# zoharl3/mantaflow

Measured on AMD Instinct MI355X. Metric: Mcells/s per step (advect+CG+FLIP), 256^3 grid, higher is better.
Workload: dtype f32; 1 GPU; 256^3 smoke step on 1 x MI355X: advectSemiLagrange(density, order 2) + advectSemiLagrange(vel, order 2) + setWallBcs + solvePressure (MIC-CG, cgAccuracy 1e-3); parallelism=single GPU

## Files before the change

### mantaflow_amd/csrc/pressure.hip

```cpp
#include "common.h"
#include "pressure.h"
#include <float.h>
#include <stdlib.h>
#include <stdio.h>
#include <type_traits>

using namespace mf;

static thread_local int g_last_shortcut[3] = {0, 0, 0};


__device__ __forceinline__ float wave_shr1(float v) {
	return __int_as_float(__builtin_amdgcn_update_dpp(__float_as_int(v), __float_as_int(v), 0x138, 0xf, 0xf, false));
}
__device__ __forceinline__ float wave_shl1(float v) {
	return __int_as_float(__builtin_amdgcn_update_dpp(__float_as_int(v), __float_as_int(v), 0x130, 0xf, 0xf, false));
}
__device__ __forceinline__ int4 unpack_flags(unsigned w) {
	return make_int4((w & 0x1u) ? MF_FLUID : 0, (w & 0x100u) ? MF_FLUID : 0, (w & 0x10000u) ? MF_FLUID : 0, (w & 0x1000000u) ? MF_FLUID : 0);
}
template <unsigned BIT>
__device__ __forceinline__ float4 unpack_coef(unsigned w) {
	return make_float4((w & BIT) ? -1.f : 0.f, (w & (BIT << 8)) ? -1.f : 0.f, (w & (BIT << 16)) ? -1.f : 0.f, (w & (BIT << 24)) ? -1.f : 0.f);
}
#ifndef AM_NT
#define AM_NT 2
#endif
#ifndef PCG_NT_MI
#define PCG_NT_MI 10
#endif
constexpr int64_t PCG_NT_CELLS = (int64_t)PCG_NT_MI << 20;
#ifndef AMP_NT
#define AMP_NT 1
#endif
template <bool DOT, bool IS3D, int R, bool PACKED>
__global__ void __launch_bounds__(BLOCK)
k_apply_matrix_v5(Dim d, const int32_t* __restrict__ flags, float* __restrict__ dst, const float* __restrict__ src,
                  const float* __restrict__ A0, const float* __restrict__ Ai, const float* __restrict__ Aj,
                  const float* __restrict__ Ak, double* __restrict__ partials, const CgScalars* __restrict__ sc, int jgroups, int tpb,
                  const unsigned char* __restrict__ pack, int dk0, int dk1, int a0p, const int* __restrict__ bempty = nullptr, int nbj = 0,
                  const int* __restrict__ outside_bad = nullptr, const int* __restrict__ xr = nullptr) {
	if (DOT && sc->done) return;
	const int qx = d.sx >> 2;
	const int64_t nthr = (int64_t)qx * jgroups * d.sz;
	const int vb0 = xcd_swizzle(blockIdx.x, gridDim.x) * tpb;
	double acc = 0.0;
#pragma unroll 1
	for (int t = 0; t < tpb; t++) {
	const int64_t T0 = (int64_t)(vb0 + t) * BLOCK + threadIdx.x;
	const bool live = T0 < nthr;
	const int64_t T = live ? T0 : nthr - 1;
	const int qi = (int)(T % qx);
	const int64_t rg = T / qx;
	const int j0 = (int)(rg % jgroups) * R;
	const int k = (int)(rg / jgroups);
	int q_lo = 0, q_hi = qx;
	if (IS3D && bempty && outside_bad[0] == 0) {
		if (xr) {
			q_lo = (xr[0] & ~7) >> 2;
			q_hi = ((xr[1] + 7) & ~7) >> 2;
		}
		if (bempty[(k >> 3) * nbj + (j0 >> 3)] || qi < q_lo || qi >= q_hi) continue;
	}
	const int lane = threadIdx.x & 63;
	const float4 z4 = make_float4(0.f, 0.f, 0.f, 0.f);
	const int64_t Y = d.Y, Z = d.Z;
	const int64_t row0 = ((int64_t)k * d.sy + j0) * d.sx + 4 * qi;
	int4 f[R];
	float4 sv[R + 2], ajv[R + 1], a0[R], ai[R], ak[R], akm[R], szm[R], szp[R];
	float sl[R], al[R], sr[R];
	{
		const int jm = (rg > 0) ? -1 : 0;
		sv[0] = *(const float4*)(src + row0 + jm * Y);
		if (PACKED) ajv[0] = unpack_coef<4u>(*(const unsigned*)(pack + row0 + jm * Y));
		else ajv[0] = *(const float4*)(Aj + row0 + jm * Y);
	}
#pragma unroll
	for (int r = 0; r < R; r++) {
		const int jr = (j0 + r < d.sy) ? r : (d.sy - 1 - j0);
		const int64_t idx = row0 + jr * Y;
		sv[r + 1] = ((AMP_NT & 1) && (!DOT || (a0p & 2))) ? ld_nt4(src + idx) : *(const float4*)(src + idx);
		unsigned pw = 0;
		if (PACKED) pw = *(const unsigned*)(pack + idx);
		if (PACKED && (a0p & 1)) a0[r] = make_float4((float)((pw >> 4) & 15u), (float)((pw >> 12) & 15u), (float)((pw >> 20) & 15u), (float)((pw >> 28) & 15u));
		else a0[r] = (AM_NT >= 1) ? ld_nt4(A0 + idx) : *(const float4*)(A0 + idx);
		if (PACKED) {
			f[r] = unpack_flags(pw);
			ajv[r + 1] = unpack_coef<4u>(pw);
			ai[r] = unpack_coef<2u>(pw);
		} else {
			f[r] = (AM_NT >= 1) ? ld_nt4i(flags + idx) : *(const int4*)(flags + idx);
			ajv[r + 1] = (AM_NT >= 3) ? ld_nt4(Aj + idx) : *(const float4*)(Aj + idx);
// ... 600 lines not shown
		else {
			lo = fminf(lo, fpart[2 * i]);
			hi = fmaxf(hi, fpart[2 * i + 1]);
		}
	}
	dd = strided_sum(dpart_dot, nbd);
	block_minmax(lo, hi);
	__syncthreads();
	ss = block_sum(ss);
	__syncthreads();
	dd = block_sum(dd);
	if (threadIdx.x == 0) {
		float resNorm;
		if (l2)
			resNorm = (float)ss;
		else {
			const float alo = fabsf(lo), ahi = fabsf(hi);
			resNorm = alo > ahi ? alo : ahi;
		}
		sc->resNorm = resNorm;
		if (resNorm < sc->accuracy) {
			sc->sigma = resNorm;
			sc->done = 1;
		} else {
			const float sigmaNew = (float)dd;
			sc->beta = sigmaNew / sc->sigma;
			sc->sigmaNew = sigmaNew;
			sc->sigma = sigmaNew;
			if (!((double)resNorm < 1e35)) {
				sc->diverged = 1;
			}
		}
	}
}
template <bool SKIP>
__global__ void __launch_bounds__(BLOCK)
k_cg_update_search_x(int64_t n, const CgScalars* __restrict__ sc, float* __restrict__ dst, float* __restrict__ search, const float* __restrict__ tmp,
                     const int* __restrict__ bempty = nullptr, int nbj = 0, int sx = 0, int sy = 0, const int* __restrict__ outside_bad = nullptr,
                     const int* __restrict__ xr = nullptr, int nt = 0) {
	if (!sc->xpending) return;
	const bool upd = !sc->done;
	const int xlo = (SKIP && xr) ? (xr[0] & ~7) : 0, xhi = (SKIP && xr) ? ((xr[1] + 7) & ~7) : 0x7fffffff;
	const float alpha = sc->alpha, beta = sc->beta;
	const int64_t n4 = n >> 2;
	const bool zero_outside = SKIP && outside_bad[0] == 0;
	for (int64_t q = blockIdx.x * (int64_t)BLOCK + threadIdx.x; q < n4; q += (int64_t)gridDim.x * BLOCK) {
		if (SKIP && zero_outside) {
			const int64_t row = (4 * q) / sx;
			const int j = (int)(row % sy), k = (int)(row / sy);
			const int xc = (int)(4 * q - row * sx);
			if (bempty[(k >> 3) * nbj + (j >> 3)] || xc < xlo || xc >= xhi) continue;
		}
		float4 s = nt ? ld_nt4(search + 4 * q) : ((float4*)search)[q];
		float4 x = nt ? ld_nt4(dst + 4 * q) : ((float4*)dst)[q];
		x.x = x.x + alpha * s.x; x.y = x.y + alpha * s.y; x.z = x.z + alpha * s.z; x.w = x.w + alpha * s.w;
		if (nt) st_nt4(dst + 4 * q, x);
		else ((float4*)dst)[q] = x;
		if (upd) {
			const float4 t = nt ? ld_nt4(tmp + 4 * q) : ((const float4*)tmp)[q];
			s.x = t.x + beta * s.x; s.y = t.y + beta * s.y; s.z = t.z + beta * s.z; s.w = t.w + beta * s.w;
			if (nt) st_nt4(search + 4 * q, s);
			else ((float4*)search)[q] = s;
		}
	}
	if (blockIdx.x == 0 && threadIdx.x < (n & 3)) {
		const int64_t i = (n4 << 2) + threadIdx.x;
		const float s = search[i];
		dst[i] = dst[i] + alpha * s;
		if (upd) search[i] = tmp[i] + beta * s;
	}
}

__global__ void __launch_bounds__(BLOCK)
k_cg_update_search_x_scalar(int64_t n, const CgScalars* __restrict__ sc, float* __restrict__ dst, float* __restrict__ search, const float* __restrict__ tmp) {
	if (!sc->xpending) return;
	const bool upd = !sc->done;
	const float alpha = sc->alpha, beta = sc->beta;
	for (int64_t i = blockIdx.x * (int64_t)BLOCK + threadIdx.x; i < n; i += (int64_t)gridDim.x * BLOCK) {
		const float s = search[i];
		dst[i] = dst[i] + alpha * s;
		if (upd) search[i] = tmp[i] + beta * s;
	}
}
__global__ void k_slab_alpha_x(const double* __restrict__ g, int world, CgScalars* __restrict__ sc, const int32_t* __restrict__ state) {
	if (state && state[0]) {
		sc->alpha = 0.f;
		sc->nalpha = -0.f;
		sc->xpending = 0;
		sc->done = 1;
		return;
	}
	double acc = 0.0;
	for (int r = 0; r < world; r++) acc += g[2 * r + 1];
	const float dp = (float)acc;
	const float a = (fabs((double)dp) > 0.) ? sc->sigma / dp : 0.f;
	sc->alpha = a;
	sc->nalpha = -a;
	sc->xpending = 1;
	sc->done = 0;
	sc->sigmaPrev = sc->sigma;
}
__global__ void __launch_bounds__(BLOCK)
k_slab_axpy_r(int64_t n, const double* __restrict__ g, int world, CgScalars* __restrict__ sc, const int32_t* __restrict__ state,
              float* __restrict__ residual, const float* __restrict__ tmp, float* __restrict__ fpart, int nt) {
	const bool stopped = state[0] != 0;
	float a = 0.f;
	if (!stopped) {
		double acc = 0.0;
		for (int r = 0; r < world; r++) acc += g[2 * r + 1];
		const float dp = (float)acc;
		a = (fabs((double)dp) > 0.) ? sc->sigma / dp : 0.f;
	}
	const float nalpha = -a;
	if (blockIdx.x == 0 && threadIdx.x == 0) {
		sc->alpha = a;
		sc->nalpha = nalpha;
		sc->xpending = stopped ? 0 : 1;
		sc->done = stopped ? 1 : 0;
		if (!stopped) sc->sigmaPrev = sc->sigma;
	}
	if (stopped) return;
	float lo = FLT_MAX, hi = -FLT_MAX;
	const int64_t n4 = n >> 2;
	for (int64_t q = blockIdx.x * (int64_t)BLOCK + threadIdx.x; q < n4; q += (int64_t)gridDim.x * BLOCK) {
		float4 r = ((float4*)residual)[q];
		const float4 t = nt ? ld_nt4(tmp + 4 * q) : ((const float4*)tmp)[q];
		r.x = r.x + nalpha * t.x; r.y = r.y + nalpha * t.y; r.z = r.z + nalpha * t.z; r.w = r.w + nalpha * t.w;
		((float4*)residual)[q] = r;
		lo = fminf(fminf(lo, r.x), fminf(r.y, fminf(r.z, r.w)));
		hi = fmaxf(fmaxf(hi, r.x), fmaxf(r.y, fmaxf(r.z, r.w)));
	}
	if (blockIdx.x == 0 && threadIdx.x < (n & 3)) {
		const int64_t i = (n4 << 2) + threadIdx.x;
		const float r = residual[i] + nalpha * tmp[i];
		residual[i] = r;
		lo = fminf(lo, r);
		hi = fmaxf(hi, r);
	}
	block_minmax(lo, hi);
	if (threadIdx.x == 0) {
		fpart[2 * blockIdx.x] = lo;
		fpart[2 * blockIdx.x + 1] = hi;
	}
}
__global__ void __launch_bounds__(BLOCK)
k_slab_axpy_r_scalar(int64_t n, const CgScalars* __restrict__ sc, float* __restrict__ residual, const float* __restrict__ tmp, float* __restrict__ fpart) {
	if (sc->done) return;
	const float nalpha = sc->nalpha;
	float lo = FLT_MAX, hi = -FLT_MAX;
	for (int64_t i = blockIdx.x * (int64_t)BLOCK + threadIdx.x; i < n; i += (int64_t)gridDim.x * BLOCK) {
		const float r = residual[i] + nalpha * tmp[i];
		residual[i] = r;
		lo = fminf(lo, r);
		hi = fmaxf(hi, r);
	}
	block_minmax(lo, hi);
	if (threadIdx.x == 0) {
		fpart[2 * blockIdx.x] = lo;
		fpart[2 * blockIdx.x + 1] = hi;
	}
}
__global__ void k_slab_beta_x(const double* __restrict__ g, int world, CgScalars* __restrict__ sc, float accuracy, int iter, int32_t* __restrict__ state) {
	if (state && state[0]) return;
	double acc = 0.0, mx = 0.0;
	for (int r = 0; r < world; r++) {
		acc += g[2 * r + 1];
		mx = g[2 * r] > mx ? g[2 * r] : mx;
	}
	const float sigmaNew = (float)acc;
	const float rn = (float)mx;
	sc->resNorm = rn;
	sc->beta = sigmaNew / sc->sigma;
	sc->sigma = sigmaNew;
	if (state) {
		if (rn < accuracy) {
			state[0] = 1;
			state[1] = iter;
			sc->done = 1;
		} else if (!(rn < 1e35f)) {
			state[0] = 2;
			state[1] = iter;
			sc->done = 1;
		}
	}
}
__global__ void __launch_bounds__(BLOCK)
k_slab_update_search_x(int64_t n, const double* __restrict__ g, int world, CgScalars* __restrict__ sc, float accuracy, int iter,
                       int32_t* __restrict__ state, float* __restrict__ dst, float* __restrict__ search, const float* __restrict__ tmp, int nt) {
	if (!sc->xpending) return;
	double acc = 0.0, mx = 0.0;
	for (int r = 0; r < world; r++) {
		acc += g[2 * r + 1];
		mx = g[2 * r] > mx ? g[2 * r] : mx;
	}
	const float sigmaNew = (float)acc;
	const float rn = (float)mx;
	const float beta = sigmaNew / sc->sigmaPrev;
	const bool converged = rn < accuracy, diverged = !converged && !(rn < 1e35f);
	if (blockIdx.x == 0 && threadIdx.x == 0) {
		sc->resNorm = rn;
		sc->beta = beta;
		sc->sigma = sigmaNew;
		if (converged || diverged) {
			state[0] = converged ? 1 : 2;
			state[1] = iter;
			sc->done = 1;
		}
	}
	const bool upd = !(converged || diverged);
	const float alpha = sc->alpha;
	const int64_t n4 = n >> 2;
	for (int64_t q = blockIdx.x * (int64_t)BLOCK + threadIdx.x; q < n4; q += (int64_t)gridDim.x * BLOCK) {
		float4 s = nt ? ld_nt4(search + 4 * q) : ((float4*)search)[q];
		float4 x = nt ? ld_nt4(dst + 4 * q) : ((float4*)dst)[q];
		x.x = x.x + alpha * s.x; x.y = x.y + alpha * s.y; x.z = x.z + alpha * s.z; x.w = x.w + alpha * s.w;
		if (nt) st_nt4(dst + 4 * q, x);
		else ((float4*)dst)[q] = x;
		if (upd) {
			const float4 t = nt ? ld_nt4(tmp + 4 * q) : ((const float4*)tmp)[q];
			s.x = t.x + beta * s.x; s.y = t.y + beta * s.y; s.z = t.z + beta * s.z; s.w = t.w + beta * s.w;
			if (nt) st_nt4(search + 4 * q, s);
			else ((float4*)search)[q] = s;
		}
	}
	if (blockIdx.x == 0 && threadIdx.x < (n & 3)) {
		const int64_t i = (n4 << 2) + threadIdx.x;
		const float s = search[i];
		dst[i] = dst[i] + alpha * s;
		if (upd) search[i] = tmp[i] + beta * s;
	}
}

__global__ void __launch_bounds__(BLOCK) k_fin_sum(int nb, const double* __restrict__ partials, double* __restrict__ out) {
	double acc = strided_sum(partials, nb);
	acc = block_sum(acc);
	if (threadIdx.x == 0) out[0] = acc;
}
__global__ void __launch_bounds__(BLOCK) k_fin_maxabs(int nb, const float* __restrict__ fpart, double* __restrict__ out) {
	float lo = FLT_MAX, hi = -FLT_MAX;
	for (int i = threadIdx.x; i < nb; i += blockDim.x) {
		lo = fminf(lo, fpart[2 * i]);
		hi = fmaxf(hi, fpart[2 * i + 1]);
	}
	block_minmax(lo, hi);
	if (threadIdx.x == 0) {
		const float alo = fabsf(lo), ahi = fabsf(hi);
		out[0] = (double)(alo > ahi ? alo : ahi);
	}
}

__global__ void __launch_bounds__(BLOCK)
k_diffusion_matrix(int64_t n, const int32_t* __restrict__ flags, float* __restrict__ A0, float* __restrict__ Ai, float* __restrict__ Aj,
                   float* __restrict__ Ak, float alpha) {
	const int64_t idx = blockIdx.x * (int64_t)BLOCK + threadIdx.x;
	if (idx >= n) return;
	if (flags[idx] & MF_OBSTACLE) {
		Ai[idx] = Aj[idx] = Ak[idx] = 0.f;
		A0[idx] = 1.f;
	} else {
		Ai[idx] *= alpha;
		Aj[idx] *= alpha;
		Ak[idx] *= alpha;
		A0[idx] = A0[idx] * alpha + 1.f;
	}
}

static int cg_solve_core(const Dim& d, const int32_t* flags, float* dst, const float* rhs, float* residual, float* search, float* tmp,
                         const float* A0, const float* Ai, const float* Aj, const float* Ak, float* Aprecond, int pc, float accuracy,
                         int maxIter, int useL2Norm, float* out_host, void* stream, const unsigned char* free_pack, const PcExternal* ext = nullptr);
__global__ void __launch_bounds__(BLOCK)
k_pad_system(int sx, int px, int64_t np_, const int32_t* __restrict__ flags, const float* __restrict__ rhs, const float* __restrict__ tmp,
             const float* __restrict__ A0, const float* __restrict__ Ai, const float* __restrict__ Aj, const float* __restrict__ Ak,
             int32_t* __restrict__ pf, float* __restrict__ pr, float* __restrict__ pt, float* __restrict__ p0, float* __restrict__ pi,
             float* __restrict__ pj, float* __restrict__ pk) {
	for (int64_t q = blockIdx.x * (int64_t)BLOCK + threadIdx.x; q < np_; q += (int64_t)gridDim.x * BLOCK) {
		const int64_t row = q / px;
		const int i = (int)(q - row * px);
		const bool in = i < sx;
		const int64_t s = row * sx + i;
		pf[q] = in ? flags[s] : MF_OBSTACLE;
		pr[q] = in ? rhs[s] : 0.f;
		pt[q] = in ? tmp[s] : 0.f;
		p0[q] = in ? A0[s] : 0.f;
		pi[q] = in ? Ai[s] : 0.f;
		pj[q] = in ? Aj[s] : 0.f;
		pk[q] = in ? Ak[s] : 0.f;
	}
}
__global__ void __launch_bounds__(BLOCK)
k_unpad(int sx, int px, int64_t n, const float* __restrict__ padded, float* __restrict__ out) {
	for (int64_t q = blockIdx.x * (int64_t)BLOCK + threadIdx.x; q < n; q += (int64_t)gridDim.x * BLOCK) {
		const int64_t row = q / sx;
		out[q] = padded[row * px + (q - row * sx)];
	}
}

static float* g_pad_buf[16];
static size_t g_pad_bytes[16];

extern "C" {

int mf_apply_matrix(int sx, int sy, int sz, const int32_t* flags, float* dst, const float* src, const float* A0,
                    const float* Ai, const float* Aj, const float* Ak, void* stream) {
	MF_TRY(check_dim(sx, sy, sz));
	const Dim d = mkdim(sx, sy, sz);
	bool a0p = false;
	const unsigned char* pk = mic_pack_user(flags, A0, Ai, Aj, Ak, &a0p);
	return launch_apply_matrix<false>(d, flags, dst, src, A0, Ai, Aj, Ak, nullptr, nullptr, (hipStream_t)stream, AmOpts{pk, a0p});
}

static int time_apply_matrix(int sx, int sy, int sz, const int32_t* flags, float* dst, const float* src, const float* A0,
                             const float* Ai, const float* Aj, const float* Ak, int reps, double* avg_us, void* stream, bool packed) {
	MF_TRY(check_dim(sx, sy, sz));
	const Dim d = mkdim(sx, sy, sz);
	hipStream_t st = (hipStream_t)stream;
	AmOpts am;
// ... 74 lines not shown
                                    const float* phi, float gfClamp, const float* curv, float surfTens, void* stream) {
	MF_TRY(check_dim(sx, sy, sz));
	const Dim d = mkdim(sx, sy, sz);
	hipLaunchKernelGGL(k_correct_velocity_gf, dim3((unsigned)((d.n + BLOCK - 1) / BLOCK)), dim3(BLOCK), 0, (hipStream_t)stream, d, vel, flags, pressure, phi, gfClamp, curv, surfTens);
	MF_LAUNCH_CHECK();
	return 0;
}
int mf_replace_clamped_ghost_fluid_vels(int sx, int sy, int sz, float* vel, const int32_t* flags, const float* pressure,
                                        const float* phi, float gfClamp, void* stream) {
	(void)pressure;
	MF_TRY(check_dim(sx, sy, sz));
	const Dim d = mkdim(sx, sy, sz);
	hipLaunchKernelGGL(k_replace_clamped_gf, dim3((unsigned)((d.n + BLOCK - 1) / BLOCK)), dim3(BLOCK), 0, (hipStream_t)stream, d, vel, flags, phi, gfClamp);
	MF_LAUNCH_CHECK();
	return 0;
}
int mf_fix_pressure(int sx, int sy, int sz, int64_t fixPidx, float value, float* rhs, float* A0, float* Ai, float* Aj, float* Ak, void* stream) {
	MF_TRY(check_dim(sx, sy, sz));
	const Dim d = mkdim(sx, sy, sz);
	if (fixPidx - d.Y < 0 || fixPidx + d.Y >= d.n || fixPidx - d.Z < 0 || fixPidx + d.Z >= d.n) return fail("fixPressure: cell %lld on the domain border", (long long)fixPidx);
	hipLaunchKernelGGL(k_fix_pressure, dim3(1), dim3(1), 0, (hipStream_t)stream, d, fixPidx, value, rhs, A0, Ai, Aj, Ak);
	MF_LAUNCH_CHECK();
	return 0;
}

int mf_apply_matrix_dot_dev(int sx, int sy, int sz, const int32_t* flags, float* dst, const float* src, const float* A0,
                            const float* Ai, const float* Aj, const float* Ak, int k0, int k1, const void* scalars, double* dot_dev,
                            void* stream) {
	MF_TRY(check_dim(sx, sy, sz));
	const Dim d = mkdim(sx, sy, sz);
	hipStream_t st = (hipStream_t)stream;
	if (k0 < 0 || k1 > sz || k0 > k1) return fail("mf_apply_matrix_dot_dev: invalid plane range");
	Workspace* ws;
	MF_TRY(get_workspace(&ws));
	const CgScalars* sc = (const CgScalars*)scalars;
	int nb = 0;
	bool ranged = false;
	AmOpts am;
	am.pack = mic_pack_user(flags, A0, Ai, Aj, Ak, &am.a0p);
	am.dk0 = k0;
	am.dk1 = k1;
	MF_TRY(launch_apply_matrix<true>(d, flags, dst, src, A0, Ai, Aj, Ak, ws->partials, sc, st, am, &nb, &ranged));
	if (!ranged) {
		const int64_t XY = (int64_t)sx * sy, n = (int64_t)(k1 - k0) * XY;
		nb = blocks_for(n >> 2, BLOCK, 2048);
		hipLaunchKernelGGL(k_cg_dot, dim3(nb), dim3(BLOCK), 0, st, n, sc, dst + k0 * XY, src + k0 * XY, ws->partials);
	}
	hipLaunchKernelGGL(k_fin_sum, dim3(1), dim3(BLOCK), 0, st, nb, ws->partials, dot_dev);
	MF_LAUNCH_CHECK();
	return 0;
}
int mf_cg_slab_axpy2(int64_t n, const void* scalars, float* x, const float* search, float* residual, const float* tmp,
                     double* maxabs_dev, void* stream) {
	if (n <= 0) return 0;
	hipStream_t st = (hipStream_t)stream;
	if (!(al16(x) && al16(search) && al16(residual) && al16(tmp))) {
		const float* alpha_dev = &((const CgScalars*)scalars)->alpha;
		MF_TRY(mf_grid_scaled_add_dev(n, x, search, alpha_dev, 1.f, stream));
		MF_TRY(mf_grid_scaled_add_dev(n, residual, tmp, alpha_dev, -1.f, stream));
		return mf_grid_max_abs_dev_f64(n, residual, maxabs_dev, stream);
	}
	Workspace* ws;
	MF_TRY(get_workspace(&ws));
	const int nb = blocks_for(n >> 2, BLOCK, 2048);
	hipLaunchKernelGGL((k_cg_axpy2<false>), dim3(nb), dim3(BLOCK), 0, st, n, (const CgScalars*)scalars, x, search, residual, (float*)tmp, ws->fpartials, ws->partials + MAX_BLOCKS);
	hipLaunchKernelGGL(k_fin_maxabs, dim3(1), dim3(BLOCK), 0, st, nb, ws->fpartials, maxabs_dev);
	MF_LAUNCH_CHECK();
	return 0;
}

int mf_diffusion_matrix(int sx, int sy, int sz, const int32_t* flags, float* A0, float* Ai, float* Aj, float* Ak, float alpha,
                        void* stream) {
	MF_TRY(check_dim(sx, sy, sz));
	const int64_t n = (int64_t)sx * sy * sz;
	hipLaunchKernelGGL(k_diffusion_matrix, dim3((unsigned)((n + BLOCK - 1) / BLOCK)), dim3(BLOCK), 0, (hipStream_t)stream, n, flags, A0, Ai, Aj, Ak, alpha);
	MF_LAUNCH_CHECK();
	return 0;
}

int mf_cg_last_shortcut(int32_t* out) {
	out[0] = g_last_shortcut[0];
	out[1] = g_last_shortcut[1];
	out[2] = g_last_shortcut[2];
	return 0;
}
int mf_cg_solve(int sx, int sy, int sz, const int32_t* flags, float* dst, const float* rhs, float* residual, float* search,
                float* tmp, const float* A0, const float* Ai, const float* Aj, const float* Ak, float* Aprecond, int pc,
                float accuracy, int maxIter, int useL2Norm, float* out_host, void* stream) {
	MF_TRY(check_dim(sx, sy, sz));
	const Dim d = mkdim(sx, sy, sz);
	hipStream_t st = (hipStream_t)stream;
	if (pc != MF_PC_NONE && pc != MF_PC_MICP) return fail("GridCg<APPLYMAT>::setICPreconditioner: Invalid method specified.");
	if (pc == MF_PC_MICP && !d.is3d) pc = MF_PC_NONE;
	if (!(al16(dst) && al16(rhs) && al16(residual) && al16(search) && al16(tmp))) return fail("mf_cg_solve: work grids must be 16-byte aligned");
	if (maxIter <= 0) {
		out_host[0] = 0.f;
		out_host[1] = 1e20f;
		out_host[2] = 0.f;
		return 0;
	}
	if (pc == MF_PC_MICP && (sx % 8) != 0 && sx >= 16) {
		const int px = (sx + 7) & ~7;
		const int64_t rows = (int64_t)sy * sz, np_ = (int64_t)px * rows;
		if (np_ < ((int64_t)1 << 31)) {
			int dev = 0;
			MF_HIP(hipGetDevice(&dev));
			float*& b = g_pad_buf[dev & 15];
			size_t& bytes = g_pad_bytes[dev & 15];
			const size_t cell = 11 * sizeof(float);
			if ((size_t)np_ * cell <= bytes || grow_buffer(&b, &bytes, cell * (size_t)(((np_ + np_ / 8 + 63) / 64) * 64), st) == 0) {
				const int64_t cap = (int64_t)(bytes / cell);
				float *p_flags = b, *p_dst = b + cap, *p_rhs = b + 2 * cap, *p_res = b + 3 * cap, *p_search = b + 4 * cap, *p_tmp = b + 5 * cap,
				      *p_A0 = b + 6 * cap, *p_Ai = b + 7 * cap, *p_Aj = b + 8 * cap, *p_Ak = b + 9 * cap, *p_Ap = b + 10 * cap;
				MF_HIP(hipMemsetAsync(p_dst, 0, sizeof(float) * np_, st));
				MF_HIP(hipMemsetAsync(p_res, 0, sizeof(float) * (cap + np_), st));
				MF_HIP(hipMemsetAsync(p_Ap, 0, sizeof(float) * np_, st));
				hipLaunchKernelGGL(k_pad_system, dim3(blocks_for(np_, BLOCK, 4096)), dim3(BLOCK), 0, st, sx, px, np_, flags, rhs, tmp, A0, Ai, Aj, Ak,
				                   (int32_t*)p_flags, p_rhs, p_tmp, p_A0, p_Ai, p_Aj, p_Ak);
				MF_LAUNCH_CHECK();
				MF_TRY(mf_cg_solve(px, sy, sz, (const int32_t*)p_flags, p_dst, p_rhs, p_res, p_search, p_tmp, p_A0, p_Ai, p_Aj, p_Ak, p_Ap, pc, accuracy,
				                   maxIter, useL2Norm, out_host, stream));
				hipLaunchKernelGGL(k_unpad, dim3(blocks_for(d.n, BLOCK, 4096)), dim3(BLOCK), 0, st, sx, px, d.n, p_dst, dst);
				MF_LAUNCH_CHECK();
				return 0;
			}
			(void)hipGetLastError();
		}
	}
	return cg_solve_core(d, flags, dst, rhs, residual, search, tmp, A0, Ai, Aj, Ak, Aprecond, pc, accuracy, maxIter, useL2Norm, out_host, stream, nullptr);
}

}

__global__ void __launch_bounds__(BLOCK)
k_pack_xrange(int64_t n, int sx, const unsigned char* __restrict__ pack, int* __restrict__ xr) {
	int lo = 0x7fffffff, hi = 0;
	const int64_t n8 = n >> 3;
	for (int64_t q = blockIdx.x * (int64_t)BLOCK + threadIdx.x; q < n8; q += (int64_t)gridDim.x * BLOCK) {
		const unsigned long long w = ((const unsigned long long*)pack)[q];
		if (w == 0ull) continue;
		const int x0 = (int)((8 * q) % sx);
		const int a = x0 + (__ffsll((long long)w) - 1) / 8, b = x0 + (63 - __clzll((long long)w)) / 8 + 2;
		lo = a < lo ? a : lo;
		hi = b > hi ? b : hi;
	}
#pragma unroll
	for (int o = 32; o >= 1; o >>= 1) {
		const int l2 = __shfl_xor(lo, o, 64), h2 = __shfl_xor(hi, o, 64);
		lo = l2 < lo ? l2 : lo;
		hi = h2 > hi ? h2 : hi;
	}
	if ((threadIdx.x & 63) == 0 && hi > 0) {
		atomicMin(&xr[0], lo);
		atomicMax(&xr[1], hi);
	}
}
__global__ void __launch_bounds__(BLOCK)
k_cg_outside_zero(int64_t n, int sx, int sy, const int* __restrict__ bempty, int nbj, const float* __restrict__ rhs, const float* __restrict__ tmp,
                  const float* __restrict__ search, int* __restrict__ bad, const int* __restrict__ xr) {
	const int64_t n4 = n >> 2;
	int found = 0;
	const int xlo = xr ? (xr[0] & ~7) : 0, xhi = xr ? ((xr[1] + 7) & ~7) : sx;
	for (int64_t q = blockIdx.x * (int64_t)BLOCK + threadIdx.x; q < n4; q += (int64_t)gridDim.x * BLOCK) {
		const int64_t row = (4 * q) / sx;
		const int j = (int)(row % sy), k = (int)(row / sy);
		const int x = (int)(4 * q - row * sx);
		if (!bempty[(k >> 3) * nbj + (j >> 3)] && x >= xlo && x < xhi) continue;
		const uint4 a = ((const uint4*)rhs)[q], b = ((const uint4*)tmp)[q], c = ((const uint4*)search)[q];
		if ((a.x | a.y | a.z | a.w | b.x | b.y | b.z | b.w | c.x | c.y | c.z | c.w) != 0u) found = 1;
	}
	if (__any(found) && (threadIdx.x & 63) == 0) atomicAdd(bad, 1);
}
struct PcgPlan {
	AmOpts am;
	const int* be_map = nullptr;
	MicSweep sweep;
};
static int pcg_setup(const Dim& d, const int32_t* flags, const float* rhs, const float* search, const float* tmp, const float* A0, const float* Ai,
                     const float* Aj, const float* Ak, const float* Aprecond, int pc, const unsigned char* free_pack, Workspace* ws, hipStream_t st,
                     PcgPlan* p) {
	const int sx = d.sx, sy = d.sy;
	const int64_t n = d.n;
	const int nbs = blocks_for(n >> 2, BLOCK, 2048);
	if (free_pack) {
		p->am.pack = free_pack;
		p->am.a0p = true;
	} else if (pc == MF_PC_MICP) {
		MF_TRY(mic_pack_query(d, flags, A0, Ai, Aj, Ak, &p->am.pack, &p->am.a0p, st));
	}
	bool several = false;
	if (pc == MF_PC_MICP && (sx % 4) == 0) MF_TRY(mic_empty_map(d, flags, Aprecond, Aj, Ak, &p->am.bempty, &p->am.nbj, &several, st));
	if (several) p->be_map = p->am.bempty;
	g_last_shortcut[0] = g_last_shortcut[1] = g_last_shortcut[2] = 0;
	p->am.nt = (!p->am.bempty && n > PCG_NT_CELLS) ? 1 : 0;
	if (p->am.bempty) {
		int* p_bad = (int*)((char*)ws->scalars + WS_PCG_FLAGS);
		int* p_xr = p_bad + 1;
		const bool ranged = p->am.pack != nullptr && (sx % 8) == 0;
		p->am.outside_bad = p_bad;
		if (ranged) p->am.xr = p_xr;
		const int init3[3] = {0, 0x7fffffff, 0};
		MF_HIP(hipMemcpyAsync(p_bad, init3, sizeof init3, hipMemcpyHostToDevice, st));
		if (ranged) hipLaunchKernelGGL(k_pack_xrange, dim3(blocks_for(n >> 3, BLOCK, 2048)), dim3(BLOCK), 0, st, n, sx, p->am.pack, p_xr);
		hipLaunchKernelGGL(k_cg_outside_zero, dim3(nbs), dim3(BLOCK), 0, st, n, sx, sy, p->am.bempty, p->am.nbj, rhs, tmp, search, p_bad, p->am.xr);
		MF_LAUNCH_CHECK();
		if (ranged) {
			int h3[3] = {1, 0, 0};
			MF_HIP(hipMemcpyAsync(h3, p_bad, sizeof h3, hipMemcpyDeviceToHost, st));
			MF_HIP(hipStreamSynchronize(st));
			int c0 = h3[1] >> 3, c1 = (h3[2] + 7) >> 3;
			if (c1 > sx / 8) c1 = sx / 8;
			if (h3[0] == 0 && h3[2] > 0 && c1 > c0) {
				p->sweep.trim_xoff = 8 * c0;
				p->sweep.trim_chunks = c1 - c0;
				g_last_shortcut[0] = 1;
				if (c1 - c0 < sx / 8) {
					g_last_shortcut[1] = 8 * c0;
					g_last_shortcut[2] = 8 * (c1 - c0);
				}
			}
		}
	}
	return 0;
}
static int cg_solve_core(const Dim& d, const int32_t* flags, float* dst, const float* rhs, float* residual, float* search, float* tmp,
                         const float* A0, const float* Ai, const float* Aj, const float* Ak, float* Aprecond, int pc, float accuracy,
                         int maxIter, int useL2Norm, float* out_host, void* stream, const unsigned char* free_pack, const PcExternal* ext) {
	const int sx = d.sx, sy = d.sy, sz = d.sz;
	const int64_t n = d.n;
	hipStream_t st = (hipStream_t)stream;
	Workspace* ws;
	MF_TRY(get_workspace(&ws));
	CgScalars* sc = (CgScalars*)ws->scalars;
	double* p_dot = ws->partials;
	double* p_res = ws->partials + MAX_BLOCKS;
	double* p_sig = ws->partials + 2 * MAX_BLOCKS;
	float* p_mm = ws->fpartials;
	const int nbs = blocks_for(n >> 2, BLOCK, 2048);

	MF_HIP(hipMemsetAsync(dst, 0, sizeof(float) * n, st));
	MF_HIP(hipMemcpyAsync(residual, rhs, sizeof(float) * n, hipMemcpyDeviceToDevice, st));
	if (pc == MF_PC_MICP) {
		if (!free_pack) MF_TRY(mf_mic_init(sx, sy, sz, flags, Aprecond, A0, Ai, Aj, Ak, stream));
		MF_TRY(mf_mic_apply(sx, sy, sz, flags, tmp, residual, Aprecond, Ai, Aj, Ak, stream));
	} else if (ext) {
		MF_TRY(ext->init(ext->ctx, A0, Ai, Aj, Ak, accuracy, st));
		MF_TRY(ext->apply(ext->ctx, tmp, residual, st));
	} else {
		MF_HIP(hipMemcpyAsync(tmp, residual, sizeof(float) * n, hipMemcpyDeviceToDevice, st));
	}
	MF_HIP(hipMemcpyAsync(search, tmp, sizeof(float) * n, hipMemcpyDeviceToDevice, st));
	MF_HIP(hipMemsetAsync(sc, 0, sizeof(CgScalars), st));
	hipLaunchKernelGGL(k_cg_dot, dim3(nbs), dim3(BLOCK), 0, st, n, sc, tmp, residual, p_sig);
	hipLaunchKernelGGL(k_cg_begin, dim3(1), dim3(BLOCK), 0, st, sc, nbs, p_sig, accuracy, useL2Norm);
	MF_LAUNCH_CHECK();
	PcgPlan p;
	MF_TRY(pcg_setup(d, flags, rhs, search, tmp, A0, Ai, Aj, Ak, Aprecond, pc, free_pack, ws, st, &p));

	CgScalars h;
	memset(&h, 0, sizeof h);
	h.resNorm = 1e20f;
	static thread_local hipEvent_t ev_dev[16][2] = {};
	int dev_ = 0;
	MF_HIP(hipGetDevice(&dev_));
	hipEvent_t* ev = ev_dev[dev_ & 15];
	if (!ev[0]) {
		MF_HIP(hipEventCreateWithFlags(&ev[0], hipEventDisableTiming));
		MF_HIP(hipEventCreateWithFlags(&ev[1], hipEventDisableTiming));
	}
	CgScalars* hslot = (CgScalars*)ws->host;
	const int batch = ((pc == MF_PC_MICP && mic_mode() == 0) || ext) ? 1 : 4;
	const int be_nb = ((sy + 7) / 8) * ((sz + 7) / 8);
	int issued = 0, slot = 0, pending = -1;
	while (issued < maxIter) {
		const int todo = (maxIter - issued < batch) ? (maxIter - issued) : batch;
		for (int it = 0; it < todo; it++) {
			int nba = 0, nsig = 0;
			bool beta_done = false;
			MF_TRY(launch_apply_matrix<true>(d, flags, tmp, search, A0, Ai, Aj, Ak, p_dot, sc, st, p.am, &nba));
			hipLaunchKernelGGL(k_cg_alpha, dim3(1), dim3(BLOCK), 0, st, sc, nba, p_dot);
			if (pc == MF_PC_MICP) {
				auto axpy = p.am.bempty ? k_cg_axpy_r<false, true> : k_cg_axpy_r<false, false>;
				hipLaunchKernelGGL(axpy, dim3(nbs), dim3(BLOCK), 0, st, n, sc, residual, tmp, p_mm, p_res, p.am.bempty, p.am.nbj, sx, sy, p_sig + be_nb,
				                   p.am.outside_bad, p.am.xr, p.am.nt);
				MicSweep fwd = p.sweep;
				MF_TRY(mic_sweep(1, d, flags, tmp, residual, Aprecond, Ai, Aj, Ak, sc, st, &fwd));
				MicSweep bwd = p.sweep;
				bwd.dotpart = p_sig;
				bwd.empty_ext = p.be_map != nullptr;
				bwd.tail = BetaTail{sc, nbs, p_mm, p_res, p.be_map ? nbs : 0};
				MF_TRY(mic_sweep(2, d, flags, tmp, residual, Aprecond, Ai, Aj, Ak, sc, st, &bwd));
				nsig = bwd.ndot;
				beta_done = bwd.tail_done;
				if (p.be_map) {
					if (nsig != be_nb) return fail("mf_cg_solve: the backward sweep wrote %d dot partials, %d expected", nsig, be_nb);
					nsig += nbs;
				}
			} else if (ext) {
				hipLaunchKernelGGL((k_cg_axpy_r<false>), dim3(nbs), dim3(BLOCK), 0, st, n, sc, residual, tmp, p_mm, p_res);
				MF_TRY(ext->apply(ext->ctx, tmp, residual, st));
			} else {
				hipLaunchKernelGGL((k_cg_axpy_r<true>), dim3(nbs), dim3(BLOCK), 0, st, n, sc, residual, tmp, p_mm, p_res);
			}
			if (nsig == 0) {
				hipLaunchKernelGGL(k_cg_dot, dim3(nbs), dim3(BLOCK), 0, st, n, sc, tmp, residual, p_sig);
				nsig = nbs;
			}
			if (!beta_done) hipLaunchKernelGGL(k_cg_beta, dim3(1), dim3(BLOCK), 0, st, sc, nbs, p_mm, p_res, nsig, p_sig);
			auto update = p.am.bempty ? k_cg_update_search_x<true> : k_cg_update_search_x<false>;
			hipLaunchKernelGGL(update, dim3(nbs), dim3(BLOCK), 0, st, n, sc, dst, search, tmp, p.am.bempty, p.am.nbj, sx, sy, p.am.outside_bad, p.am.xr, p.am.nt);
		}
		MF_LAUNCH_CHECK();
		issued += todo;
		MF_HIP(hipMemcpyAsync(&hslot[slot], sc, sizeof(CgScalars), hipMemcpyDeviceToHost, st));
		MF_HIP(hipEventRecord(ev[slot], st));
		if (ext) pending = slot;
		if (pending >= 0) {
			MF_HIP(hipEventSynchronize(ev[pending]));
			memcpy(&h, &hslot[pending], sizeof h);
			if (h.done || h.diverged) break;
		}
		pending = slot;
		slot ^= 1;
	}
	MF_HIP(hipMemcpyAsync(&hslot[0], sc, sizeof(CgScalars), hipMemcpyDeviceToHost, st));
	MF_HIP(hipStreamSynchronize(st));
	memcpy(&h, &hslot[0], sizeof h);
	out_host[0] = (float)h.iterations;
	out_host[1] = h.resNorm;
	out_host[2] = h.sigma;
	if (pc == MF_PC_MICP) MF_TRY(mic_flow_error());
	if (h.diverged) return fail("GridCg::iterate: The CG solver diverged, residual norm > 1e30, stopping.");
	return 0;
}

namespace mf {
int cg_solve_external(const Dim& d, const int32_t* flags, float* dst, const float* rhs, float* residual, float* search, float* tmp,
                      const float* A0, const float* Ai, const float* Aj, const float* Ak, const PcExternal* ext, float accuracy, int maxIter,
                      int useL2Norm, float* out_host, void* stream) {
	if (!(al16(dst) && al16(rhs) && al16(residual) && al16(search) && al16(tmp))) return fail("cg_solve_external: work grids must be 16-byte aligned");
	if (maxIter <= 0) {
		out_host[0] = 0.f;
		out_host[1] = 1e20f;
		out_host[2] = 0.f;
		return 0;
	}
	return cg_solve_core(d, flags, dst, rhs, residual, search, tmp, A0, Ai, Aj, Ak, nullptr, MF_PC_MGP, accuracy, maxIter, useL2Norm, out_host, stream,
	                     nullptr, ext);
}
}

__global__ void __launch_bounds__(BLOCK)
k_setup_fused(Dim d, const int32_t* __restrict__ flags, const float* __restrict__ vel, float* __restrict__ rhs, unsigned char* __restrict__ pack,
              int* __restrict__ bempty, int nbj) {
	const int qx = d.sx >> 2;
	const int64_t T = blockIdx.x * (int64_t)BLOCK + threadIdx.x;
	if (T >= (int64_t)qx * d.sy * d.sz) return;
	const int qi = (int)(T % qx);
	const int64_t rg = T / qx;
	const int j = (int)(rg % d.sy), k = (int)(rg / d.sy), i0 = 4 * qi;
	const int64_t Y = d.Y, Z = d.Z, n = d.n;
	const int64_t idx = i0 + Y * j + Z * k;
	const int4 f4 = *(const int4*)(flags + idx);
	const int f[4] = {f4.x, f4.y, f4.z, f4.w};
	float r[4] = {0.f, 0.f, 0.f, 0.f};
	unsigned bytes = 0;
	const bool row_in = j >= 1 && j <= d.sy - 2 && k >= 1 && k <= d.sz - 2;
	if (row_in) {
		const int4 ym4 = *(const int4*)(flags + idx - Y), yp4 = *(const int4*)(flags + idx + Y);
		const int4 zm4 = *(const int4*)(flags + idx - Z), zp4 = *(const int4*)(flags + idx + Z);
		const int ym[4] = {ym4.x, ym4.y, ym4.z, ym4.w}, yp[4] = {yp4.x, yp4.y, yp4.z, yp4.w};
		const int zm[4] = {zm4.x, zm4.y, zm4.z, zm4.w}, zp[4] = {zp4.x, zp4.y, zp4.z, zp4.w};
		const int fxm = i0 > 0 ? flags[idx - 1] : MF_OBSTACLE, fxp = i0 + 4 < d.sx ? flags[idx + 4] : MF_OBSTACLE;
		const float *vx = vel, *vy = vel + n, *vz = vel + 2 * n;
		const float4 ux4 = *(const float4*)(vx + idx), uy4 = *(const float4*)(vy + idx), uyp4 = *(const float4*)(vy + idx + Y);
		const float4 uz4 = *(const float4*)(vz + idx), uzp4 = *(const float4*)(vz + idx + Z);
		const float uxp = i0 + 4 < d.sx ? vx[idx + 4] : 0.f;
		const float ux[5] = {ux4.x, ux4.y, ux4.z, ux4.w, uxp};
		const float uy[4] = {uy4.x, uy4.y, uy4.z, uy4.w}, uyp[4] = {uyp4.x, uyp4.y, uyp4.z, uyp4.w};
		const float uz[4] = {uz4.x, uz4.y, uz4.z, uz4.w}, uzp[4] = {uzp4.x, uzp4.y, uzp4.z, uzp4.w};
#pragma unroll
		for (int c = 0; c < 4; c++) {
			const int i = i0 + c;
			const bool fl = (f[c] & MF_FLUID) != 0;
			unsigned b = fl ? 1u : 0u;
			if (fl && i >= 1 && i <= d.sx - 2) {
				const int xm = c > 0 ? f[c - 1] : fxm, xp = c < 3 ? f[c + 1] : fxp;
				const unsigned a0 = (unsigned)!(xm & MF_OBSTACLE) + (unsigned)!(xp & MF_OBSTACLE) + (unsigned)!(ym[c] & MF_OBSTACLE) +
				                    (unsigned)!(yp[c] & MF_OBSTACLE) + (unsigned)!(zm[c] & MF_OBSTACLE) + (unsigned)!(zp[c] & MF_OBSTACLE);
				b |= ((xp & MF_FLUID) ? 2u : 0u) | ((yp[c] & MF_FLUID) ? 4u : 0u) | ((zp[c] & MF_FLUID) ? 8u : 0u) | (a0 << 4);
				float set = ux[c] - ux[c + 1] + uy[c] - uyp[c];
				set += uz[c] - uzp[c];
				r[c] = set;
			}
			bytes |= b << (8 * c);
		}
	} else {
#pragma unroll
		for (int c = 0; c < 4; c++) bytes |= ((f[c] & MF_FLUID) ? 1u : 0u) << (8 * c);
	}
	*(float4*)(rhs + idx) = make_float4(r[0], r[1], r[2], r[3]);
	*(unsigned*)(pack + idx) = bytes;
	if (bytes & 0x01010101u) bempty[(k >> 3) * nbj + (j >> 3)] = 0;
}

extern "C" {
// ... 84 lines not shown
```

Before: 237.4 Mcells/s.

## Fuse CG search/x update into next iteration's matrix-apply kernel with ping-pong buffers

Adds a fused kernel that computes the new search direction s = z + beta*s_old on the fly, applies the packed 7-point matrix to it, updates x += alpha*s_old, writes s_new and Ap, and produces dot partials. Stencil neighbours are rebuilt from z and s_old. The separate update_search_x pass is dropped for every iteration after the first, and double-buffered search/tmp arrays let reads and writes go to different storage. This saves a full-grid read/write sweep per CG iteration, at the price of recomputing neighbour search values, higher register pressure, an extra scratch allocation, and one trailing update after the loop.

```diff
diff --git a/mantaflow_amd/csrc/pressure.hip b/mantaflow_amd/csrc/pressure.hip
--- a/mantaflow_amd/csrc/pressure.hip
+++ b/mantaflow_amd/csrc/pressure.hip
@@ -8,6 +8,7 @@
 using namespace mf;
 
 static thread_local int g_last_shortcut[3] = {0, 0, 0};
+static thread_local int g_last_fused = 0;
 
 
 __device__ __forceinline__ float wave_shr1(float v) {
@@ -774,6 +775,169 @@
 		if (upd) search[i] = tmp[i] + beta * s;
 	}
 }
+
+__device__ __forceinline__ float4 search_upd4(float4 t, float beta, float4 s) {
+	return make_float4(t.x + beta * s.x, t.y + beta * s.y, t.z + beta * s.z, t.w + beta * s.w);
+}
+template <int R>
+__global__ void __launch_bounds__(BLOCK)
+k_cg_search_apply(Dim d, const CgScalars* __restrict__ sc, float* __restrict__ x, const float* __restrict__ so, const float* __restrict__ zz,
+                  float* __restrict__ sn, float* __restrict__ ap, const unsigned char* __restrict__ pack, double* __restrict__ partials,
+                  int jgroups, int tpb, int nt) {
+	if (!sc->xpending) return;
+	const bool upd = !sc->done;
+	const float alpha = sc->alpha, beta = sc->beta;
+	const int qx = d.sx >> 2;
+	const int64_t nthr = (int64_t)qx * jgroups * d.sz;
+	const int vb0 = xcd_swizzle(blockIdx.x, gridDim.x) * tpb;
+	const int64_t Y = d.Y, Z = d.Z;
+	if (!upd) {
+		for (int t = 0; t < tpb; t++) {
+			const int64_t T = (int64_t)(vb0 + t) * BLOCK + threadIdx.x;
+			if (T >= nthr) break;
+			const int64_t rg = T / qx;
+			const int j0 = (int)(rg % jgroups) * R;
+			const int64_t row0 = ((rg / jgroups) * d.sy + j0) * d.sx + 4 * (T % qx);
+			for (int r = 0; r < R && j0 + r < d.sy; r++) {
+				const int64_t idx = row0 + r * Y;
+				const float4 s = nt ? ld_nt4(so + idx) : *(const float4*)(so + idx);
+				float4 xv = nt ? ld_nt4(x + idx) : *(const float4*)(x + idx);
+				xv.x = xv.x + alpha * s.x; xv.y = xv.y + alpha * s.y; xv.z = xv.z + alpha * s.z; xv.w = xv.w + alpha * s.w;
+				if (nt) st_nt4(x + idx, xv);
+				else *(float4*)(x + idx) = xv;
+			}
+		}
+		return;
+	}
+	double acc = 0.0;
+#pragma unroll 1
+	for (int t = 0; t < tpb; t++) {
+	const int64_t T0 = (int64_t)(vb0 + t) * BLOCK + threadIdx.x;
+	const bool live = T0 < nthr;
+	const int64_t T = live ? T0 : nthr - 1;
+	const int qi = (int)(T % qx);
+	const int64_t rg = T / qx;
+	const int j0 = (int)(rg % jgroups) * R;
+	const int k = (int)(rg / jgroups);
+	const int lane = threadIdx.x & 63;
+	const float4 z4 = make_float4(0.f, 0.f, 0.f, 0.f);
+	const int64_t row0 = ((int64_t)k * d.sy + j0) * d.sx + 4 * qi;
+	int4 f[R];
+	float4 sv[R + 2], ajv[R + 1], a0[R], ai[R], ak[R], akm[R], szm[R], szp[R], xo[R], own_s[R];
+	float sl[R], al[R], sr[R];
+	{
+		const int64_t im = row0 + ((rg > 0) ? -Y : 0);
+		sv[0] = search_upd4(*(const float4*)(zz + im), beta, *(const float4*)(so + im));
+		ajv[0] = unpack_coef<4u>(*(const unsigned*)(pack + im));
+	}
+#pragma unroll
+	for (int r = 0; r < R; r++) {
+		const int jr = (j0 + r < d.sy) ? r : (d.sy - 1 - j0);
+		const int64_t idx = row0 + jr * Y;
+		const float4 s = nt ? ld_nt4(so + idx) : *(const float4*)(so + idx);
+		const float4 tz = nt ? ld_nt4(zz + idx) : *(const float4*)(zz + idx);
+		xo[r] = nt ? ld_nt4(x + idx) : *(const float4*)(x + idx);
+		own_s[r] = s;
+		sv[r + 1] = search_upd4(tz, beta, s);
+		const unsigned pw = *(const unsigned*)(pack + idx);
+		a0[r] = make_float4((float)((pw >> 4) & 15u), (float)((pw >> 12) & 15u), (float)((pw >> 20) & 15u), (float)((pw >> 28) & 15u));
+		f[r] = unpack_flags(pw);
+		ajv[r + 1] = unpack_coef<4u>(pw);
+		ai[r] = unpack_coef<2u>(pw);
+		const int64_t im = (k > 0) ? idx - Z : idx, ip = (k < d.sz - 1) ? idx + Z : idx;
+		ak[r] = unpack_coef<8u>(pw);
+		akm[r] = unpack_coef<8u>(*(const unsigned*)(pack + im));
+		szm[r] = search_upd4(*(const float4*)(zz + im), beta, *(const float4*)(so + im));
+		szp[r] = search_upd4(*(const float4*)(zz + ip), beta, *(const float4*)(so + ip));
+	}
+	{
+		const int jr = (j0 + R < d.sy) ? R : (d.sy - j0 - ((k < d.sz - 1) ? 0 : 1));
+		sv[R + 1] = search_upd4(*(const float4*)(zz + row0 + jr * Y), beta, *(const float4*)(so + row0 + jr * Y));
+	}
+	const bool edge_l = (lane == 0) || (qi == 0), edge_r = (lane == 63) || (qi == qx - 1);
+#pragma unroll
+	for (int r = 0; r < R; r++) {
+		const int jr = (j0 + r < d.sy) ? r : (d.sy - 1 - j0);
+		const int64_t idx = row0 + jr * Y;
+		sl[r] = wave_shr1(sv[r + 1].w);
+		al[r] = wave_shr1(ai[r].w);
+		sr[r] = wave_shl1(sv[r + 1].x);
+		if (edge_l) {
+			sl[r] = (idx > 0) ? (zz[idx - 1] + beta * so[idx - 1]) : 0.f;
+			al[r] = (idx > 0 && (pack[idx - 1] & 2u)) ? -1.f : 0.f;
+		}
+		if (edge_r) sr[r] = (idx + 4 < d.n) ? (zz[idx + 4] + beta * so[idx + 4]) : 0.f;
+	}
+#pragma unroll
+	for (int r = 0; r < R; r++) {
+		const int j = j0 + r;
+		if (j >= d.sy) break;
+		const int4 fl = f[r];
+		const float4 s = sv[r + 1];
+		float4 res = s;
+		if ((fl.x | fl.y | fl.z | fl.w) & MF_FLUID) {
+			const float4 sym = (j > 0 || k > 0) ? sv[r] : z4, ajm = (j > 0 || k > 0) ? ajv[r] : z4;
+			const float4 syp = (j < d.sy - 1) ? sv[r + 2] : (k < d.sz - 1) ? sv[R + 1] : z4, aj = ajv[r + 1];
+			float4 zm = z4, am = z4, zp = z4;
+			const float4 akc = ak[r];
+			if (k > 0) {
+				zm = szm[r];
+				am = akm[r];
+			}
+			if (k < d.sz - 1) zp = szp[r];
+#define CELL5(c, SL, AL, SR)                                                                      \
+	if (fl.c & MF_FLUID) {                                                                        \
+		float v = s.c * a0[r].c;                                                                  \
+		v = v + (SL) * (AL);                                                                      \
+		v = v + (SR) * ai[r].c;                                                                   \
+		v = v + sym.c * ajm.c;                                                                    \
+		v = v + syp.c * aj.c;                                                                     \
+		v = v + zm.c * am.c;                                                                      \
+		v = v + zp.c * akc.c;                                                                     \
+		res.c = v;                                                                                \
+	}
+			CELL5(x, sl[r], al[r], s.y)
+			CELL5(y, s.x, ai[r].x, s.z)
+			CELL5(z, s.y, ai[r].y, s.w)
+			CELL5(w, s.z, ai[r].z, sr[r])
+#undef CELL5
+		}
+		if (live) {
+			float4 xv = xo[r];
+			const float4 os = own_s[r];
+			xv.x = xv.x + alpha * os.x; xv.y = xv.y + alpha * os.y; xv.z = xv.z + alpha * os.z; xv.w = xv.w + alpha * os.w;
+			if (nt) {
+				st_nt4(x + row0 + r * Y, xv);
+				st_nt4(sn + row0 + r * Y, s);
+				st_nt4(ap + row0 + r * Y, res);
+			} else {
+				*(float4*)(x + row0 + r * Y) = xv;
+				*(float4*)(sn + row0 + r * Y) = s;
+				*(float4*)(ap + row0 + r * Y) = res;
+			}
+			const float p0 = res.x * s.x, p1 = res.y * s.y, p2 = res.z * s.z, p3 = res.w * s.w;
+			acc += (double)p0;
+			acc += (double)p1;
+			acc += (double)p2;
+			acc += (double)p3;
+		}
+	}
+	}
+	acc = block_sum(acc);
+	if (threadIdx.x == 0) partials[blockIdx.x] = acc;
+}
+static int launch_search_apply(const Dim& d, const CgScalars* sc, float* x, const float* s_old, const float* z, float* s_new, float* Ap,
+                               const unsigned char* pack, double* partials, int nt, hipStream_t st, int* nblocks) {
+	constexpr int R = 2;
+	const int jgroups = (d.sy + R - 1) / R;
+	const int64_t vblocks = ((int64_t)(d.sx >> 2) * jgroups * d.sz + BLOCK - 1) / BLOCK;
+	const int tpb = (int)((vblocks + MAX_BLOCKS - 1) / MAX_BLOCKS);
+	const int nb = (int)((vblocks + tpb - 1) / tpb);
+	hipLaunchKernelGGL(k_cg_search_apply<R>, dim3(nb), dim3(BLOCK), 0, st, d, sc, x, s_old, z, s_new, Ap, pack, partials, jgroups, tpb, nt);
+	MF_LAUNCH_CHECK();
+	if (nblocks) *nblocks = nb;
+	return 0;
+}
 __global__ void k_slab_alpha_x(const double* __restrict__ g, int world, CgScalars* __restrict__ sc, const int32_t* __restrict__ state) {
 	if (state && state[0]) {
 		sc->alpha = 0.f;
@@ -924,6 +1088,12 @@
 }
 
 __global__ void __launch_bounds__(BLOCK) k_fin_sum(int nb, const double* __restrict__ partials, double* __restrict__ out) {
+	double acc = strided_sum(partials, nb);
+	acc = block_sum(acc);
+	if (threadIdx.x == 0) out[0] = acc;
+}
+__global__ void __launch_bounds__(BLOCK) k_cg_fused_dot_fin(const CgScalars* __restrict__ sc, int nb, const double* __restrict__ partials, double* __restrict__ out) {
+	if (!sc->xpending || sc->done) return;
 	double acc = strided_sum(partials, nb);
 	acc = block_sum(acc);
 	if (threadIdx.x == 0) out[0] = acc;
@@ -1164,6 +1334,28 @@
 	out[0] = g_last_shortcut[0];
 	out[1] = g_last_shortcut[1];
 	out[2] = g_last_shortcut[2];
+	return 0;
+}
+int mf_cg_last_fused(int32_t* out) {
+	out[0] = g_last_fused;
+	return 0;
+}
+int mf_cg_search_apply_pass(int sx, int sy, int sz, const int32_t* flags, const float* A0, const float* Ai, const float* Aj, const float* Ak,
+                            const void* scalars, float* x, const float* s_old, const float* z, float* s_new, float* Ap, double* dot_dev,
+                            int nt, void* stream) {
+	MF_TRY(check_dim(sx, sy, sz));
+	const Dim d = mkdim(sx, sy, sz);
+	hipStream_t st = (hipStream_t)stream;
+	bool a0p = false;
+	const unsigned char* pack = mic_pack_user(flags, A0, Ai, Aj, Ak, &a0p);
+	if (!pack || !a0p || !d.is3d || (sx % 4) != 0) return fail("mf_cg_search_apply_pass: needs a 3-D system with sx %% 4 == 0 packed by mf_pack_matrix, diagonal included");
+	if (!(al16(x) && al16(s_old) && al16(z) && al16(s_new) && al16(Ap))) return fail("mf_cg_search_apply_pass: grids must be 16-byte aligned");
+	Workspace* ws;
+	MF_TRY(get_workspace(&ws));
+	int nb = 0;
+	MF_TRY(launch_search_apply(d, (const CgScalars*)scalars, x, s_old, z, s_new, Ap, pack, ws->partials, nt, st, &nb));
+	hipLaunchKernelGGL(k_cg_fused_dot_fin, dim3(1), dim3(BLOCK), 0, st, (const CgScalars*)scalars, nb, ws->partials, dot_dev);
+	MF_LAUNCH_CHECK();
 	return 0;
 }
 int mf_cg_solve(int sx, int sy, int sz, const int32_t* flags, float* dst, const float* rhs, float* residual, float* search,
@@ -1305,6 +1497,12 @@
 	}
 	return 0;
 }
+static float* g_fuse_buf[16];
+static size_t g_fuse_bytes[16];
+static bool pcg_fuse_wanted() {
+	const char* e = getenv("MF_PCG_FUSE");
+	return !(e && e[0] == '0');
+}
 static int cg_solve_core(const Dim& d, const int32_t* flags, float* dst, const float* rhs, float* residual, float* search, float* tmp,
                          const float* A0, const float* Ai, const float* Aj, const float* Ak, float* Aprecond, int pc, float accuracy,
                          int maxIter, int useL2Norm, float* out_host, void* stream, const unsigned char* free_pack, const PcExternal* ext) {
@@ -1353,13 +1551,39 @@
 	CgScalars* hslot = (CgScalars*)ws->host;
 	const int batch = ((pc == MF_PC_MICP && mic_mode() == 0) || ext) ? 1 : 4;
 	const int be_nb = ((sy + 7) / 8) * ((sz + 7) / 8);
+	float* S[2] = {search, nullptr};
+	float* T[2] = {tmp, nullptr};
+	int par = 0;
+	bool fuse = pcg_fuse_wanted() && pc == MF_PC_MICP && d.is3d && p.am.pack && p.am.a0p && !p.am.bempty && p.am.nt == 0 && (sx % 4) == 0 &&
+	            al16(flags) && al16(dst) && al16(search) && al16(tmp) && al16(A0) && al16(Ai) && al16(Aj) && al16(Ak);
+	if (fuse) {
+		float*& b = g_fuse_buf[dev_ & 15];
+		size_t& bytes = g_fuse_bytes[dev_ & 15];
+		const size_t cell = 2 * sizeof(float);
+		if ((size_t)n * cell <= bytes || grow_buffer(&b, &bytes, cell * (size_t)(((n + n / 8 + 63) / 64) * 64), st) == 0) {
+			S[1] = b;
+			T[1] = b + bytes / cell;
+		} else {
+			(void)hipGetLastError();
+			fuse = false;
+		}
+	}
+	g_last_fused = fuse ? 1 : 0;
+	auto update = p.am.bempty ? k_cg_update_search_x<true> : k_cg_update_search_x<false>;
 	int issued = 0, slot = 0, pending = -1;
 	while (issued < maxIter) {
 		const int todo = (maxIter - issued < batch) ? (maxIter - issued) : batch;
 		for (int it = 0; it < todo; it++) {
 			int nba = 0, nsig = 0;
 			bool beta_done = false;
-			MF_TRY(launch_apply_matrix<true>(d, flags, tmp, search, A0, Ai, Aj, Ak, p_dot, sc, st, p.am, &nba));
+			if (fuse && issued + it > 0) {
+				MF_TRY(launch_search_apply(d, sc, dst, S[par], T[par], S[par ^ 1], T[par ^ 1], p.am.pack, p_dot, p.am.nt, st, &nba));
+				par ^= 1;
+			} else {
+				MF_TRY(launch_apply_matrix<true>(d, flags, T[par], S[par], A0, Ai, Aj, Ak, p_dot, sc, st, p.am, &nba));
+			}
+			float* const search = S[par];
+			float* const tmp = T[par];
 			hipLaunchKernelGGL(k_cg_alpha, dim3(1), dim3(BLOCK), 0, st, sc, nba, p_dot);
 			if (pc == MF_PC_MICP) {
 				auto axpy = p.am.bempty ? k_cg_axpy_r<false, true> : k_cg_axpy_r<false, false>;
@@ -1389,8 +1613,7 @@
 				nsig = nbs;
 			}
 			if (!beta_done) hipLaunchKernelGGL(k_cg_beta, dim3(1), dim3(BLOCK), 0, st, sc, nbs, p_mm, p_res, nsig, p_sig);
-			auto update = p.am.bempty ? k_cg_update_search_x<true> : k_cg_update_search_x<false>;
-			hipLaunchKernelGGL(update, dim3(nbs), dim3(BLOCK), 0, st, n, sc, dst, search, tmp, p.am.bempty, p.am.nbj, sx, sy, p.am.outside_bad, p.am.xr, p.am.nt);
+			if (!fuse) hipLaunchKernelGGL(update, dim3(nbs), dim3(BLOCK), 0, st, n, sc, dst, search, tmp, p.am.bempty, p.am.nbj, sx, sy, p.am.outside_bad, p.am.xr, p.am.nt);
 		}
 		MF_LAUNCH_CHECK();
 		issued += todo;
@@ -1404,6 +1627,10 @@
 		}
 		pending = slot;
 		slot ^= 1;
+	}
+	if (fuse) {
+		hipLaunchKernelGGL(update, dim3(nbs), dim3(BLOCK), 0, st, n, sc, dst, S[par], T[par], p.am.bempty, p.am.nbj, sx, sy, p.am.outside_bad, p.am.xr, p.am.nt);
+		MF_LAUNCH_CHECK();
 	}
 	MF_HIP(hipMemcpyAsync(&hslot[0], sc, sizeof(CgScalars), hipMemcpyDeviceToHost, st));
 	MF_HIP(hipStreamSynchronize(st));
```

Measured after the change: 237.1 Mcells/s. About the same (-0.2%).
